# Xjh-UCAS/TAM-TR

Measured on AMD Instinct MI355X. Metric: images/sec fwd+bwd @640x640 bs=16/GPU, higher is better.
Workload: dtype bf16

## Files before the change

### include/tamtr_hip.h

```cpp
#ifndef TAMTR_HIP_H
#define TAMTR_HIP_H

#include <stdint.h>

#ifdef __cplusplus
extern "C" {
#endif

#define TAMTR_F32 0
#define TAMTR_BF16 1

#define TAMTR_OK 0
#define TAMTR_EINVAL (-1)
#define TAMTR_EUNSUP (-2)
#define TAMTR_ELAUNCH (-3)

int tamtr_abi_version(void);

int tamtr_maxsigmoid_gate_fwd(const void* x, const float* gk, const float* bias, const void* v, void* out, float* aw,
                              int32_t* arg, int B, int nh, int hc, int HW, int T, float scale, int dtype, void* stream);

int tamtr_maxsigmoid_gate_bwd(const void* dout, const void* x, const float* gk, const void* v, const float* aw,
                              const int32_t* arg, void* dx, void* dv, float* dlogit, int B, int nh, int hc, int HW, int T,
                              float scale, int dtype, void* stream);
// ... 13 lines not shown
int tamtr_msdeform_attn_fwd(const void* value, const int32_t* shapes_host, const float* loc, const float* aw, void* out,
                            int B, int L, int M, int D, int Q, int nl, int P, int dtype, void* stream);

int tamtr_msdeform_attn_bwd(const void* gout, const void* value, const int32_t* shapes_host, const float* loc,
                            const float* aw, float* gvalue, float* gloc, float* gaw, int B, int L, int M, int D, int Q,
                            int nl, int P, int dtype, void* stream);

int tamtr_msdeform_attn_bwd_sorted(const void* gout, const void* value, const int32_t* shapes_host, const float* loc,
                                   const float* aw, void* gvalue, float* gloc, float* gaw, float* colw, int B, int L, int M,
                                   int D, int Q, int nl, int P, long long ldg, int dtype, void* stream);

int tamtr_contrastive_logits_fwd(const void* x, const float* w, const float* logit_scale, const float* bias, float* logits,
                                 float* xinv, float* winv, int B, int Q, int K, int C, int dtype, void* stream);

int tamtr_contrastive_bwd_slabs(int Q);
int tamtr_contrastive_logits_bwd(const float* g, const void* x, const float* w, const float* logit_scale, const float* xinv,
                                 const float* winv, void* dx, float* dwhat, int B, int Q, int K, int C, int dtype,
                                 void* stream);

int tamtr_linear_bf16(const void* X, const void* W, const float* bias, void* Y, int M, int N, int K, void* stream);

int tamtr_selfattn_fwd(const void* q, const void* k, const void* v, const uint32_t* mask_bits, void* o, float* lse, int B,
                       int Q, int nh, int dh, int ldq, int ldk, int ldv, int dtype, void* stream);
int tamtr_selfattn_bwd(const void* go, const void* q, const void* k, const void* v, const void* o, const float* lse,
                       const uint32_t* mask_bits, void* gq, void* gk, void* gv, float* delta_ws, int B, int Q, int nh, int dh,
                       int ldq, int ldk, int ldv, int dtype, void* stream);

int tamtr_selective_scan_chunk(void);
int tamtr_selective_scan_fwd(const float* u, const float* delta, const float* A, const float* Bm, const float* Cm,
                             const float* D, const float* dbias, float* y, float* hstate, int B, int K, int Dk, int N, int L,
                             int xmode, void* stream);
int tamtr_selective_scan_bwd_slabs(int Dk);
int tamtr_selective_scan_row_sums(void);
int tamtr_selective_scan_bwd(const float* gy, const float* u, const float* delta, const float* A, const float* Bm,
                             const float* Cm, const float* D, const float* dbias, const float* hstate, float* gu,
                             float* gdelta, float* grow, float* gB, float* gC, float* ws, int B, int K, int Dk, int N, int L,
                             int xmode, void* stream);

int tamtr_selective_scan_dtproj_fwd(const void* u, const float* dtr, const float* Wdt, const float* A, const float* Bm,
                                    const float* Cm, const float* D, const float* dbias, void* y, float* hstate, int B, int K,
                                    int Dk, int N, int R, int L, int xmode, int planes_bf16, void* stream);
int tamtr_selective_scan_dtproj_bwd(const void* gy, const void* u, const float* dtr, const float* Wdt, const float* A,
                                    const float* Bm, const float* Cm, const float* D, const float* dbias, const float* hstate,
                                    void* gu, void* gdelta_ws, float* gdtr, float* grow, float* gB, float* gC, float* ws, int B,
                                    int K, int Dk, int N, int R, int L, int xmode, int bf16_flags, void* stream);

int tamtr_lsap_assign(const float* cost, const int32_t* group_sizes_host, int bs, int nq, int G, int64_t* batch_idx,
                      int64_t* query_idx, int64_t* gt_idx, void* stream);

int tamtr_cpam_fwd(const void* x, const void* p, void* out, float* s2, int32_t* arg, int B, int C, int H, int W, int dtype,
                   void* stream);

int tamtr_cpam_bwd(const void* gout, const void* x, const void* p, const float* s2, const int32_t* arg, void* dx_direct,
                   void* du_ws, void* dp, int B, int C, int H, int W, int dtype, void* stream);

int tamtr_cpam_cl_fwd(const void* x, void* p, uint8_t* code, void* out, float* s2, int32_t* arg, int B, int C, int H, int W, int dtype, void* stream);
int tamtr_cpam_cl_bwd(const void* gout, const void* x, const void* p, const uint8_t* code, const float* s2, const int32_t* arg, void* dxd_ws,
                      void* du_ws, void* dp_ws, void* dx, int B, int C, int H, int W, int dtype, void* stream);

int tamtr_dwconv_silu_cross_fwd(const void* x, long long x_pixel_stride, const float* weight, const float* bias, void* u2, int B,
                                int D, int H, int W, int dtype, int plane_dtype, void* stream);
int tamtr_dwconv_tiles(int H, int W);
int tamtr_dwconv_silu_cross_bwd(const void* g2, const void* x, long long x_pixel_stride, const float* weight, const float* bias,
                                void* gx, long long gx_pixel_stride, float* ws, int B, int D, int H, int W, int dtype, int plane_dtype,
                                void* stream);

int tamtr_cross_merge_fwd(const void* y4, float* ymT, int B, int D, int H, int W, int plane_dtype, void* stream);
int tamtr_cross_merge_bwd(const float* gymT, void* g2, int B, int D, int H, int W, int plane_dtype, void* stream);

int tamtr_ln_gate_blocks(long long ntok);
int tamtr_ln_gate_fwd(const float* x, const void* xz, long long xz_token_stride, const float* gamma, const float* beta, void* out,
                      float* stats, long long ntok, int D, float eps, int dtype, void* stream);
int tamtr_ln_gate_bwd(const void* gout, const float* x, const void* xz, long long xz_token_stride, const float* gamma,
                      const float* beta, const float* stats, float* gx, void* gxz, float* partials, long long ntok, int D, int dtype,
                      void* stream);

int tamtr_sum_n(const void* const* src, int n, void* out, long long n_elems, int dtype, void* stream);

int tamtr_colsum_blocks(long long M);
int tamtr_colsum_bf16(const void* X, float* partial, long long M, int N, void* stream);
int tamtr_slab_sum_rows(const void* in, float* out, int R, long long C, int dtype, void* stream);
int tamtr_dw_slices(long long M, int N, int K);
int tamtr_dw_bf16(const void* dY, const void* X, float* part, int with_db, long long M, int N, int K, void* stream);
int tamtr_fold_add(const float* g4, const void* m0, const void* m1, float* out, int B, long long n, int dtype, void* stream);

int tamtr_layernorm_fwd(const void* x, const float* gamma, const float* beta, void* out, float* stats, long long ntok, int D,
                        float eps, int dtype, void* stream);
int tamtr_layernorm_bwd(const void* gout, const void* x, const float* gamma, const float* stats, void* gx, float* partials,
                        long long ntok, int D, int dtype, void* stream);

int tamtr_bn_slices(int B, int HW);
int tamtr_bn_act_fwd(const void* x, const float* gamma, const float* beta, float* running_mean, float* running_var, void* y,
                     float* mean_rstd, float* partials, int B, int C, int HW, float eps, float momentum, int act, int dtype, void* stream);
int tamtr_bn_act_bwd(const void* gy, const void* x, const float* gamma, const float* beta, const float* mean_rstd, void* gx,
                     float* ggamma, float* gbeta, float* partials, int B, int C, int HW, int act, int dtype, void* stream);

int tamtr_bncl_blocks(long long N, int C, int dtype);
int tamtr_bncl_act_fwd(const void* x, const float* gamma, const float* beta, float* running_mean, float* running_var, const void* residual,
                       void* y, float* mean_rstd, float* partials, long long N, int C, float eps, float momentum, int act, int dtype,
                       void* stream);
int tamtr_bncl_stats(const void* x, float* running_mean, float* running_var, float* mean_rstd, float* partials, long long N, int C, float eps,
                     float momentum, int dtype, void* stream);
int tamtr_bncl2_act_fwd(const void* x1, const float* gamma1, const float* beta1, float* running_mean1, float* running_var1, const void* x2,
                        const float* gamma2, const float* beta2, float* running_mean2, float* running_var2, void* y, float* mean_rstd,
                        float* partials, long long N, int C, float eps, float momentum, int act, int dtype, void* stream);
int tamtr_bncl2_act_bwd(const void* gy, long long ldgy, const void* x1, const void* x2, const float* gamma1, const float* beta1,
                        const float* gamma2, const float* beta2, const float* mean_rstd, void* gx1, void* gx2, float* ggamma1, float* gbeta1,
                        float* ggamma2, float* gbeta2, float* partials, long long N, int C, int act, int dtype, void* stream);
int tamtr_bncl_act_bwd(const void* gy, long long ldgy, const void* x, const float* gamma, const float* beta, const float* mean_rstd,
                       void* gx, float* ggamma, float* gbeta, float* partials, long long N, int C, int act, int dtype, void* stream);
int tamtr_bncl_act_down2_fwd(const void* x, const float* gamma, const float* beta, float* running_mean, float* running_var, void* y,
                             float* mean_rstd, float* partials, int B, int H, int W, int C, float eps, float momentum, int act, int dtype,
                             void* stream);
int tamtr_bncl_act_down2_bwd(const void* gy, long long ldgy, const void* x, const float* gamma, const float* beta, const float* mean_rstd,
                             void* gx, float* ggamma, float* gbeta, float* partials, int B, int H, int W, int C, int act, int dtype,
                             void* stream);

int tamtr_relayout(const void* src, void* dst, int B, int C, int HW, int ld, int to_nhwc, int dtype, void* stream);
int tamtr_resample2(const void* src, void* dst, int B, int H, int W, int C, int mode, int dtype, void* stream);
int tamtr_copy_rows(const void* src, long long lds, void* dst, long long ldd, long long N, int C, int dtype, void* stream);
int tamtr_cat_rows(const void* const* src, const long long* lds, const int* C, int n, void* dst, long long ldd, long long N, int dtype,
                   void* stream);

int tamtr_maxpool_out(int n, int k, int s, int p);
int tamtr_maxpool_fwd(const void* x, void* y, uint8_t* code, int B, int C, int H, int W, int k, int s, int p, int nhwc, int dtype,
                      void* stream);
int tamtr_maxpool_bwd(const void* gy, const uint8_t* code, const void* addend, void* gx, int B, int C, int H, int W, int k, int s, int p, int nhwc, int dtype,
                      void* stream);

int tamtr_img_augment_u8(const uint8_t* src, const double* inv_affine, const uint8_t* luts, const int32_t* flags, float* out, int B,
                         int SH, int SW, int H, int W, int border, void* stream);

int tamtr_optim_chunk(void);
int tamtr_optim_step(const void* const* p, const void* const* m, const void* const* v, const void* const* e, const void* const* shadow, float* step,
                     const long long* numel,
                     const unsigned char* group, const int* chunk_tensor, const long long* chunk_off, const void* const* grads, int ntensors,
                     int nchunks, float* partial, float* normcoef, const float* lr, const float* wd, int ngroups, float beta1, float beta2, float eps,
                     float max_norm, float ema_decay, int do_ema, void* stream);

int tamtr_xproj_dw_slices(int L);
int tamtr_xproj_fwd(const void* u2, const void* wcat, float* dtr, float* Bs, float* Cs, int B, int D, int L, int R, int plane_dtype, void* stream);
int tamtr_xproj_bwd_dx(const void* gu, const float* gdtr, const float* gB, const float* gC, const void* wT, void* gu2, int B, int D, int L, int R,
                       int plane_dtype, void* stream);
int tamtr_xproj_bwd_dw(const void* u2, const float* gdtr, const float* gB, const float* gC, float* part, int B, int D, int L, int R, int plane_dtype,
                       void* stream);

int tamtr_detr_blocks(int rows_per_layer);
int tamtr_detr_layers_fwd(const float* pb, const float* ps, const float* gt_bboxes, const long long* gt_cls, const long long* li, const long long* bi,
                          const long long* si, const long long* gi, int Lr, int B, int nq, int nc, int n, long long* tgt, float* score, float* pair_l1,
                          float* pair_riou, float* partial, float g_class, float g_bbox, float g_giou, float* out, void* stream);
int tamtr_detr_layers_bwd(const float* pb, const float* ps, const float* gt_bboxes, const long long* li, const long long* bi, const long long* si,
                          const long long* gi, const long long* tgt, const float* score, const float* up, int Lr, int B, int nq, int nc, int n,
                          float g_class, float g_bbox, float g_giou, float* gpb, float* gps, void* stream);
int tamtr_detr_match_cost(const float* ps, const float* pb, const float* gt_bboxes, const long long* gt_cls, long long rows, int nc, int G, float g_class,
                          float g_bbox, float g_giou, float alpha, float gamma, float* C, void* stream);

int tamtr_bncl_act_seg_fwd(const void* x, const float* gamma, const float* beta, float* running_mean, float* running_var, void* y, long long seg_rows,
                           long long seg_pitch, float* mean_rstd, float* partials, long long N, int C, float eps, float momentum, int act, int dtype,
                           void* stream);
int tamtr_bncl_act_seg_bwd(const void* gy, long long seg_rows, long long seg_pitch, const void* x, const float* gamma, const float* beta,
                           const float* mean_rstd, void* gx, float* ggamma, float* gbeta, float* partials, long long N, int C, int act, int dtype,
                           void* stream);

int tamtr_box_refine_fwd(const float* delta, const float* ref, float* out, long long n, void* stream);
int tamtr_box_refine_bwd(const float* gout, const float* out, const float* ref, float* gdelta, float* gref, long long n, void* stream);

// ... 129 lines not shown
```

### tam-tr_amd/_lib.py

```python
import ctypes
import os
from ctypes import c_float, c_int, c_longlong, c_void_p

_HERE = os.path.dirname(os.path.abspath(__file__))
LIB_PATH = os.environ.get('TAMTR_HIP_LIB') or os.path.join(_HERE, 'csrc', 'libtamtr_hip.so')
ABI_VERSION = 36

F32, BF16 = 0, 1
_ERR = {-1: 'TAMTR_EINVAL (bad argument)', -2: 'TAMTR_EUNSUP (shape/dtype outside what the kernels are built for)',
        -3: 'TAMTR_ELAUNCH (HIP launch error)'}


class TamtrHipError(RuntimeError):
    pass


_P, _I, _F, _LL, _D = c_void_p, c_int, c_float, c_longlong, ctypes.c_double
_SIGS = {
    'tamtr_abi_version': [],
    'tamtr_maxsigmoid_gate_fwd': [_P, _P, _P, _P, _P, _P, _P, _I, _I, _I, _I, _I, _F, _I, _P],
    'tamtr_maxsigmoid_gate_bwd': [_P, _P, _P, _P, _P, _P, _P, _P, _P, _I, _I, _I, _I, _I, _F, _I, _P],
    'tamtr_msdeform_attn_fwd': [_P, _P, _P, _P, _P, _I, _I, _I, _I, _I, _I, _I, _I, _P],
    'tamtr_msdeform_attn_bwd': [_P, _P, _P, _P, _P, _P, _P, _P, _I, _I, _I, _I, _I, _I, _I, _I, _P],
    'tamtr_msdeform_attn_bwd_sorted': [_P, _P, _P, _P, _P, _P, _P, _P, _P, _I, _I, _I, _I, _I, _I, _I, _LL, _I, _P],
    'tamtr_contrastive_logits_fwd': [_P, _P, _P, _P, _P, _P, _P, _I, _I, _I, _I, _I, _P],
    'tamtr_contrastive_logits_bwd': [_P, _P, _P, _P, _P, _P, _P, _P, _I, _I, _I, _I, _I, _P],
    'tamtr_contrastive_bwd_slabs': [_I],
    'tamtr_linear_bf16': [_P, _P, _P, _P, _I, _I, _I, _P],
    'tamtr_selfattn_fwd': [_P, _P, _P, _P, _P, _P, _I, _I, _I, _I, _I, _I, _I, _I, _P],
    'tamtr_selfattn_bwd': [_P] * 11 + [_I, _I, _I, _I, _I, _I, _I, _I, _P],
    'tamtr_selective_scan_chunk': [],
    'tamtr_selective_scan_fwd': [_P, _P, _P, _P, _P, _P, _P, _P, _P, _I, _I, _I, _I, _I, _I, _P],
    'tamtr_selective_scan_bwd_slabs': [_I],
    'tamtr_selective_scan_row_sums': [],
    'tamtr_selective_scan_bwd': [_P] * 15 + [_I, _I, _I, _I, _I, _I, _P],
    'tamtr_selective_scan_dtproj_fwd': [_P] * 10 + [_I] * 8 + [_P],
    'tamtr_selective_scan_dtproj_bwd': [_P] * 17 + [_I] * 8 + [_P],
    'tamtr_lsap_assign': [_P, _P, _I, _I, _I, _P, _P, _P, _P],
    'tamtr_img_augment_u8': [_P, _P, _P, _P, _P, _I, _I, _I, _I, _I, _I, _P],
    'tamtr_cpam_fwd': [_P, _P, _P, _P, _P, _I, _I, _I, _I, _I, _P],
    'tamtr_cpam_cl_fwd': [_P, _P, _P, _P, _P, _P, _I, _I, _I, _I, _I, _P],
    'tamtr_cpam_bwd': [_P] * 8 + [_I, _I, _I, _I, _I, _P],
    'tamtr_cpam_cl_bwd': [_P] * 10 + [_I, _I, _I, _I, _I, _P],
    'tamtr_dwconv_silu_cross_fwd': [_P, _LL, _P, _P, _P, _I, _I, _I, _I, _I, _I, _P],
    'tamtr_dwconv_tiles': [_I, _I],
    'tamtr_cross_merge_fwd': [_P, _P, _I, _I, _I, _I, _I, _P],
    'tamtr_cross_merge_bwd': [_P, _P, _I, _I, _I, _I, _I, _P],
    'tamtr_ln_gate_blocks': [_LL],
    'tamtr_bn_slices': [_I, _I],
    'tamtr_maxpool_out': [_I, _I, _I, _I],
    'tamtr_maxpool_fwd': [_P, _P, _P, _I, _I, _I, _I, _I, _I, _I, _I, _I, _P],
    'tamtr_maxpool_bwd': [_P, _P, _P, _P, _I, _I, _I, _I, _I, _I, _I, _I, _I, _P],
    'tamtr_sum_n': [_P, _I, _P, _LL, _I, _P],
    'tamtr_colsum_blocks': [_LL],
    'tamtr_colsum_bf16': [_P, _P, _LL, _I, _P],
    'tamtr_fold_add': [_P, _P, _P, _P, _I, _LL, _I, _P],
    'tamtr_slab_sum_rows': [_P, _P, _I, _LL, _I, _P],
    'tamtr_dw_slices': [_LL, _I, _I],
    'tamtr_dw_bf16': [_P, _P, _P, _I, _LL, _I, _I, _P],
    'tamtr_graph_capture_census': [_P, _P, _I],
    'tamtr_box_refine_fwd': [_P, _P, _P, _LL, _P],
    'tamtr_box_refine_bwd': [_P, _P, _P, _P, _P, _LL, _P],
    'tamtr_bncl_act_seg_fwd': [_P, _P, _P, _P, _P, _P, _LL, _LL, _P, _P, _LL, _I, _F, _F, _I, _I, _P],
    'tamtr_bncl_act_seg_bwd': [_P, _LL, _LL, _P, _P, _P, _P, _P, _P, _P, _P, _LL, _I, _I, _I, _P],
    'tamtr_detr_blocks': [_I],
    'tamtr_detr_layers_fwd': [_P] * 8 + [_I] * 5 + [_P] * 5 + [_F, _F, _F, _P, _P],
    'tamtr_detr_layers_bwd': [_P] * 10 + [_I] * 5 + [_F, _F, _F, _P, _P, _P],
    'tamtr_detr_match_cost': [_P, _P, _P, _P, _LL, _I, _I, _F, _F, _F, _F, _F, _P, _P],
    'tamtr_xproj_dw_slices': [_I],
    'tamtr_xproj_fwd': [_P, _P, _P, _P, _P, _I, _I, _I, _I, _I, _P],
    'tamtr_xproj_bwd_dx': [_P, _P, _P, _P, _P, _P, _I, _I, _I, _I, _I, _P],
    'tamtr_xproj_bwd_dw': [_P, _P, _P, _P, _P, _I, _I, _I, _I, _I, _P],
    'tamtr_optim_chunk': [],
    'tamtr_optim_step': [_P] * 11 + [_I, _I, _P, _P, _P, _P, _I, _F, _F, _F, _F, _F, _I, _P],
    'tamtr_resample2': [_P, _P, _I, _I, _I, _I, _I, _I, _P],
    'tamtr_cat_rows': [_P, _P, _P, _I, _P, _LL, _LL, _I, _P],
    'tamtr_copy_rows': [_P, _LL, _P, _LL, _LL, _I, _I, _P],
    'tamtr_relayout': [_P, _P, _I, _I, _I, _I, _I, _I, _P],
    'tamtr_bncl_blocks': [_LL, _I, _I],
    'tamtr_bncl_act_fwd': [_P, _P, _P, _P, _P, _P, _P, _P, _P, _LL, _I, _F, _F, _I, _I, _P],
    'tamtr_bncl_stats': [_P, _P, _P, _P, _P, _LL, _I, _F, _F, _I, _P],
    'tamtr_bn_finalize': [_P, _P, _P, _P, _I, _I, _F, _F, _P],
    'tamtr_conv3x3_tiles': [_I, _I, _I],
    'tamtr_conv3x3_pack_weight': [_P, _P, _I, _I, _I, _P],
    'tamtr_conv3x3_cl_stats_fwd': [_P, _LL, _P, _P, _P, _P, _P, _P, _I, _I, _I, _I, _I, _F, _F, _P],
    'tamtr_maxsigmoid_gate_cl_fwd': [_P, _LL, _P, _P, _P, _P, _P, _P, _P, _P, _P, _P, _P, _P, _I, _I, _I, _I, _I, _F, _I, _P],
    'tamtr_bncl2_act_fwd': [_P, _P, _P, _P, _P, _P, _P, _P, _P, _P, _P, _P, _P, _LL, _I, _F, _F, _I, _I, _P],
    'tamtr_bncl2_act_bwd': [_P, _LL, _P, _P, _P, _P, _P, _P, _P, _P, _P, _P, _P, _P, _P, _P, _LL, _I, _I, _I, _P],
    'tamtr_bncl_act_bwd': [_P, _LL, _P, _P, _P, _P, _P, _P, _P, _P, _LL, _I, _I, _I, _P],
    'tamtr_bncl_act_down2_fwd': [_P, _P, _P, _P, _P, _P, _P, _P, _I, _I, _I, _I, _F, _F, _I, _I, _P],
    'tamtr_bncl_act_down2_bwd': [_P, _LL, _P, _P, _P, _P, _P, _P, _P, _P, _I, _I, _I, _I, _I, _I, _P],
    'tamtr_bn_act_fwd': [_P, _P, _P, _P, _P, _P, _P, _P, _I, _I, _I, _F, _F, _I, _I, _P],
    'tamtr_bn_act_bwd': [_P, _P, _P, _P, _P, _P, _P, _P, _P, _I, _I, _I, _I, _I, _P],
    'tamtr_layernorm_fwd': [_P, _P, _P, _P, _P, _LL, _I, _F, _I, _P],
    'tamtr_layernorm_bwd': [_P, _P, _P, _P, _P, _P, _LL, _I, _I, _P],
    'tamtr_ln_gate_fwd': [_P, _P, _LL, _P, _P, _P, _P, _LL, _I, _F, _I, _P],
    'tamtr_ln_gate_bwd': [_P, _P, _P, _LL, _P, _P, _P, _P, _P, _P, _LL, _I, _I, _P],
    'tamtr_dwconv_silu_cross_bwd': [_P, _P, _LL, _P, _P, _P, _LL, _P, _I, _I, _I, _I, _I, _I, _P],
    'tamtr_detect_postprocess': [_P, _I, _I, _I, _I, _P, _F, _F, _I, _F, _P, _I, _P, _P, _P, _P],
    'tamtr_val_postprocess_match': [_P, _I, _I, _I, _I, _F, _F, _F, _I, _F, _P, _P, _P, _I, _P, _P, _P, _P, _P],
    'tamtr_val_confusion': [_P, _P, _I, _I, _I, _P, _P, _P, _I, _P, _F, _F, _P, _P],
    'tamtr_val_ap_tile': [],
    'tamtr_val_ap_curves': [_P, _P, _P, _I, _I, _P, _I] + [_P] * 10 + [_P],
    'tamtr_text_embed': [_P, _P, _P, _P, _LL, _I, _I, _I, _P],
    'tamtr_linear_f32': [_P, _P, _P, _P, _P, _I, _I, _I, _I, _P],
    'tamtr_text_pool_project': [_P, _P, _P, _P, _P, _P, _I, _I, _I, _I, _F, _I, _P],
    'tamtr_bytetrack_update': [_P, _P, _I, _I, _P, _P, _P, _P, _P, _I, _F, _F, _F, _D, _I, _P, _P, _P, _I, _P],
    'tamtr_bytetrack_workspace_bytes': [_I, _I],
    'tamtr_botsort_update': [_P, _P, _P, _I, _I, _P, _P, _P, _P, _P, _I, _F, _F, _F, _D, _I, _P, _P, _P, _I, _P],
    'tamtr_botsort_reid_update': [_P, _P, _P, _P, _I, _I, _P, _P, _P, _P, _P, _P, _I, _I, _F, _F, _F, _D, _I, _F, _D, _P, _P, _P, _I, _P],
    'tamtr_botsort_reid_workspace_bytes': [_I, _I],
    'tamtr_reid_rows': [_P, _I, _P, _P, _I, _I, _I, _I, _P, _P],
    'tamtr_gmc_workspace_bytes': [_I, _I, _I],
    'tamtr_gmc_workspace_offset': [_I, _I, _I, _I],
    'tamtr_gmc_state_bytes': [_I, _I],
    'tamtr_gmc_estimate': [_P, _P, _P, _I, _I, _I, _P, _P, _P, _P, _P, _P, _I, _I, _P],
    'tamtr_bytetrack_update_streams': [_P, _P, _I, _I, _I, _P, _P, _P, _P, _P, _I, _F, _F, _F, _D, _I, _P, _P, _P, _I, _P],
    'tamtr_bytetrack_streams_workspace_bytes': [_I, _I, _I],
    'tamtr_botsort_update_streams': [_P, _P, _P, _I, _I, _I, _P, _P, _P, _P, _P, _I, _F, _F, _F, _D, _I, _P, _P, _P, _I, _P],
    'tamtr_botsort_reid_update_streams': [_P, _P, _P, _P, _I, _I, _I, _P, _P, _P, _P, _P, _P, _I, _I, _F, _F, _F, _D, _I, _F, _D, _P, _P, _P, _I,
                                          _P],
    'tamtr_botsort_reid_streams_workspace_bytes': [_I, _I, _I],
    'tamtr_gmc_estimate_streams': [_P, _P, _P, _I, _I, _I, _I, _P, _P, _P, _P, _P, _P, _I, _I, _P],
    'tamtr_val_coco_match': [_P, _P, _I, _I, _I, _P, _P, _P, _I, _P, _P, _I, _P, _P, _P, _P, _I, _P],
    'tamtr_val_coco_workspace_bytes': [_I, _I, _I],
    'tamtr_val_coco_accumulate': [_P, _P, _P, _I, _I, _P, _P, _I, _P, _P, _P, _P, _P],
    'tamtr_mot_update': [_P, _P, _P, _P, _I, _I, _I, _I, _D, _P, _P, _P, _P, _P, _I, _I, _P, _I, _P],
    'tamtr_mot_end_sequence': [_I, _P, _P, _P, _P, _I, _I, _I, _P, _I, _P],
    'tamtr_mot_workspace_bytes': [_I, _I, _I, _I, _I],
    'tamtr_hota_update': [_P, _P, _P, _P, _I, _I, _I, _I, _D, _D, _P, _P, _P, _I, _P],
    'tamtr_hota_end_sequence': [_P, _D, _I, _I, _I, _I, _P, _P, _P, _I, _P],
    'tamtr_hota_workspace_bytes': [_I, _I, _I],
    'tamtr_mot_update_streams': [_P, _P, _P, _P, _I, _I, _I, _I, _I, _D, _P, _P, _P, _P, _P, _P, _I, _I, _P, _I, _P],
    'tamtr_mot_end_streams': [_I, _I, _P, _P, _P, _P, _P, _P, _I, _I, _P, _I, _P],
    'tamtr_mot_streams_workspace_bytes': [_I, _I, _I, _I, _I, _I],
    'tamtr_hota_update_streams': [_P, _P, _P, _P, _I, _I, _I, _I, _I, _D, _D, _P, _P, _P, _P, _I, _P],
    'tamtr_hota_end_streams': [_P, _D, _I, _I, _P, _I, _I, _I, _P, _P, _P, _I, _P],
    'tamtr_hota_streams_workspace_bytes': [_I, _I, _I, _I],
    'tamtr_trackmap_update': [_P, _P, _P, _P, _I, _I, _I, _I, _D, _P, _P, _P, _I, _P],
    'tamtr_trackmap_end_sequence': [_P, _I, _D, _I, _P, _P, _P, _I, _P],
    'tamtr_trackmap_workspace_bytes': [_I, _I, _I, _I, _I, _I],
    'tamtr_tta_view': [_P, _P, _I, _I, _I, _I, _I, _I, _I, _I, _P],
# ... 78 lines not shown
```

### tam-tr_amd/csrc/dwgrad.hip

```cpp
#include "common.h"

namespace {

constexpr int DW_T = 256;
constexpr int DW_ROWS = 64;
constexpr int DW_RB = 128;
constexpr int DW_SMAX = 64;
constexpr int DW_MIN_ROWS = 256;
constexpr int DW_FILL = 512;

__device__ __forceinline__ uint32_t dswz(int row, int chunk) { return (uint32_t)row * DW_RB + (uint32_t)((chunk ^ ((row ^ (row >> 3)) & 7)) << 4); }

template <int TN, int TK>
__global__ __launch_bounds__(DW_T, 2) void dw_bf16_kernel(const bf16_t* __restrict__ dY, const bf16_t* __restrict__ X, float* __restrict__ part,
                                                           int with_db, long long M, int N, int K, long long rps, int n_tiles, int k_tiles, int S, long long pitch) {
  extern __shared__ __attribute__((aligned(16))) unsigned char smem[];
  constexpr int ST_BYTES = (TN + TK) * DW_RB;
  constexpr int NI = TN / 64, KI = TK / 64;
  const int tid = threadIdx.x, lane = tid & 63, wave = tid >> 6;
  const int wn = wave >> 1, wk = wave & 1;
  const int lr = lane & 31, lh = lane >> 5;
  const int xcd = blockIdx.x & 7, slot = blockIdx.x >> 3;
  int sl, nt, kt;
  if (S >= 8) {
    const int tiles = n_tiles * k_tiles, t = slot % tiles;
    sl = (slot / tiles) * 8 + xcd; nt = t / k_tiles; kt = t % k_tiles;
  } else {
    const int unit = (slot / k_tiles) * 8 + xcd;
    sl = unit / n_tiles; nt = unit % n_tiles; kt = slot % k_tiles;
  }
  if (sl >= S) return;
  const int n0 = nt * TN, k0 = kt * TK;
  const long long m_lo = (long long)sl * rps;
  const long long m_hi = m_lo + rps < M ? m_lo + rps : M;
  const int nst = (int)((m_hi - m_lo + DW_ROWS - 1) / DW_ROWS);

  const bool isY = tid < TN, has_task = tid < TN + TK;
  const int u = isY ? tid : tid - TN;
  const int cpr = (isY ? TN : TK) / 8;
  const int c = u % cpr, rg = u / cpr;
  const int ld = isY ? N : K;
  const int col = (isY ? n0 : k0) + 8 * c;
  const bool col_ok = has_task && col < ld;
  const bf16_t* src = (isY ? dY : X) + (col_ok ? col : 0);
  const long long mrow = m_lo + rg * 8;
  unsigned char* sdst = smem + (isY ? 0 : TN * DW_RB);
  const bool do_db = with_db && kt == 0 && isY;

  uint4 r[8];
  unsigned live = 0;
  float colacc[8];
#pragma unroll
  for (int j = 0; j < 8; ++j) colacc[j] = 0.f;

  auto g_load = [&](int st) {
    const long long m = mrow + (long long)st * DW_ROWS;
    live = 0;
#pragma unroll
    for (int i = 0; i < 8; ++i) {
      const bool in = m + i < m_hi;
      r[i] = *reinterpret_cast<const uint4*>(src + (size_t)(in ? m + i : m_hi - 1) * ld);
      live |= (col_ok && in ? 1u : 0u) << i;
    }
  };
  auto s_store = [&](int stage) {
    if (!has_task) return;
#pragma unroll
    for (int i = 0; i < 8; ++i)
      if (!((live >> i) & 1)) r[i] = make_uint4(0, 0, 0, 0);
    if (do_db) {
#pragma unroll
      for (int i = 0; i < 8; ++i) {
        const uint32_t d[4] = {r[i].x, r[i].y, r[i].z, r[i].w};
#pragma unroll
        for (int q = 0; q < 4; ++q) {
          colacc[2 * q] += __uint_as_float(d[q] << 16);
          colacc[2 * q + 1] += __uint_as_float(d[q] & 0xffff0000u);
        }
      }
    }
    unsigned char* base = sdst + stage * ST_BYTES;
#pragma unroll
    for (int q = 0; q < 4; ++q) {
      uint32_t lo[4], hi[4];
#pragma unroll
      for (int e = 0; e < 4; ++e) {
        const uint32_t a = q == 0 ? r[2 * e].x : q == 1 ? r[2 * e].y : q == 2 ? r[2 * e].z : r[2 * e].w;
        const uint32_t b = q == 0 ? r[2 * e + 1].x : q == 1 ? r[2 * e + 1].y : q == 2 ? r[2 * e + 1].z : r[2 * e + 1].w;
        lo[e] = (a & 0xffffu) | (b << 16);
        hi[e] = (a >> 16) | (b & 0xffff0000u);
      }
      *reinterpret_cast<uint4*>(base + dswz(8 * c + 2 * q, rg)) = make_uint4(lo[0], lo[1], lo[2], lo[3]);
      *reinterpret_cast<uint4*>(base + dswz(8 * c + 2 * q + 1, rg)) = make_uint4(hi[0], hi[1], hi[2], hi[3]);
    }
  };

  f32x16 acc[NI][KI];
#pragma unroll
  for (int a = 0; a < NI; ++a)
#pragma unroll
    for (int b = 0; b < KI; ++b)
#pragma unroll
      for (int q = 0; q < 16; ++q) acc[a][b][q] = 0.f;

  g_load(0);
  s_store(0);
  __syncthreads();
  for (int st = 0; st < nst; ++st) {
    const int cur = st & 1;
    if (st + 1 < nst) g_load(st + 1);
    const unsigned char* sy = smem + cur * ST_BYTES;
    const unsigned char* sx = sy + TN * DW_RB;
#pragma unroll
    for (int ks = 0; ks < DW_ROWS / 16; ++ks) {
      const int ch = ks * 2 + lh;
      s16x8 fy[NI], fx[KI];
#pragma unroll
      for (int i = 0; i < NI; ++i) fy[i] = *reinterpret_cast<const s16x8*>(sy + dswz(wn * (TN / 2) + i * 32 + lr, ch));
#pragma unroll
      for (int j = 0; j < KI; ++j) fx[j] = *reinterpret_cast<const s16x8*>(sx + dswz(wk * (TK / 2) + j * 32 + lr, ch));
#pragma unroll
      for (int i = 0; i < NI; ++i)
#pragma unroll
        for (int j = 0; j < KI; ++j) acc[i][j] = __builtin_amdgcn_mfma_f32_32x32x16_bf16(fy[i], fx[j], acc[i][j], 0, 0, 0);
    }
    if (st + 1 < nst) {
      s_store(cur ^ 1);
      __syncthreads();
    }
  }

  float* out = part + (size_t)sl * pitch;
#pragma unroll
  for (int i = 0; i < NI; ++i)
#pragma unroll
    for (int j = 0; j < KI; ++j) {
      const int k = k0 + wk * (TK / 2) + j * 32 + lr;
#pragma unroll
      for (int q = 0; q < 16; ++q) {
        const int n = n0 + wn * (TN / 2) + i * 32 + (q & 3) + 8 * (q >> 2) + 4 * lh;
        if (n < N && k < K) out[(size_t)n * K + k] = acc[i][j][q];
      }
    }

  if (kt == 0) {
    float* red = reinterpret_cast<float*>(smem);
    __syncthreads();
    if (do_db) {
#pragma unroll
      for (int j = 0; j < 8; ++j) red[rg * TN + 8 * c + j] = colacc[j];
    }
    __syncthreads();
    if (tid < TN && n0 + tid < N) {
      float s = 0.f;
      if (with_db) {
#pragma unroll
        for (int g = 0; g < 8; ++g) s += red[g * TN + tid];
      }
      out[(size_t)N * K + n0 + tid] = s;
    }
  }
}

struct DwPlan {
  int tn, tk, n_tiles, k_tiles, S;
  long long rps;
};

long long dw_rows_per_slice(long long M, int S) { return ((M + S - 1) / S + DW_ROWS - 1) / DW_ROWS * DW_ROWS; }

bool dw_plan(long long M, int N, int K, DwPlan* p) {
  if (M <= 0 || N <= 0 || K <= 0 || N % 16 || K % 16 || N > 16384 || K > 16384 || M > (1LL << 40)) return false;
  long long smax = M / DW_MIN_ROWS;
  smax = smax < 1 ? 1 : smax > DW_SMAX ? DW_SMAX : smax;
  int tn = N >= 128 ? 128 : 64, tk = K >= 128 ? 128 : 64;
  auto tiles = [&]() { return (long long)((N + tn - 1) / tn) * ((K + tk - 1) / tk); };
  if (tiles() * smax < DW_FILL / 2) tn = tk = 64;
  const long long t = tiles();
  long long S = (DW_FILL + t - 1) / t;
  S = S < 1 ? 1 : S > smax ? smax : S;
  for (;;) {
    const long long rows = dw_rows_per_slice(M, (int)S), s2 = (M + rows - 1) / rows;
    if (s2 == S) break;
    S = s2;
  }
  p->tn = tn; p->tk = tk;
  p->n_tiles = (N + tn - 1) / tn; p->k_tiles = (K + tk - 1) / tk;
  p->S = (int)S;
  p->rps = dw_rows_per_slice(M, (int)S);
  return true;
}

}

extern "C" int tamtr_dw_slices(long long M, int N, int K) {
  DwPlan p;
  return dw_plan(M, N, K, &p) ? p.S : 0;
}

extern "C" int tamtr_dw_bf16(const void* dY, const void* X, float* part, int with_db, long long M, int N, int K, void* stream) {
  if (!dY || !X || !part || M <= 0 || N <= 0 || K <= 0) return TAMTR_EINVAL;
  DwPlan p;
  if (!dw_plan(M, N, K, &p)) return TAMTR_EUNSUP;
  if (((uintptr_t)dY | (uintptr_t)X | (uintptr_t)part) % 16) return TAMTR_EUNSUP;
  const long long pitch = (long long)N * K + (N + 3) / 4 * 4;
  const int groups = p.S >= 8 ? (p.S + 7) / 8 * p.n_tiles * p.k_tiles : (p.S * p.n_tiles + 7) / 8 * p.k_tiles;
  const dim3 grid((unsigned)groups * 8);
  const size_t lds = (size_t)2 * (p.tn + p.tk) * DW_RB;
#define LAUNCH_DW(TN_, TK_)                                                                                                       \
  hipLaunchKernelGGL((dw_bf16_kernel<TN_, TK_>), grid, dim3(DW_T), lds, (hipStream_t)stream, (const bf16_t*)dY, (const bf16_t*)X, \
                     part, with_db, M, N, K, p.rps, p.n_tiles, p.k_tiles, p.S, pitch)
  if (p.tn == 128 && p.tk == 128) LAUNCH_DW(128, 128);
  else if (p.tn == 128) LAUNCH_DW(128, 64);
  else if (p.tk == 128) LAUNCH_DW(64, 128);
  else LAUNCH_DW(64, 64);
#undef LAUNCH_DW
  return tamtr_launch_status();
}
```

### tam-tr_amd/ops.py

```python
import ctypes
import math

import torch

from . import _lib
from ._lib import call, dtype_code, ptr, require_gpu, stream_ptr
import os as _os

_PROJ_CONV_LIB = _os.environ.get('TAMTR_PROJ_CONV') == 'miopen'

_I, _F = ctypes.c_int, ctypes.c_float


def _c(t):
    return t if t.is_contiguous() else t.contiguous()


def _is_cl(t):
    return t.dim() == 4 and not t.is_contiguous() and t.is_contiguous(memory_format=torch.channels_last)


def is_cl(t):
    return _is_cl(t)

# ... 373 lines not shown
        D = N // M
        Q = loc32.shape[1]
        gout = _c(gout.to(torch.bfloat16))
        gloc, gaw = torch.empty_like(loc32), torch.empty_like(aw32)
        colw = torch.empty(B, Q, M, device=gout.device, dtype=torch.float32)
        gvalue = torch.empty(B * L, N, device=gout.device, dtype=torch.bfloat16)
        call('tamtr_msdeform_attn_bwd_sorted', ptr(gout), ptr(value), ctypes.cast(sh, ctypes.c_void_p), ptr(loc32), ptr(aw32),
             ptr(gvalue), ptr(gloc), ptr(gaw), ptr(colw), B, L, M, D, Q, nl, P, N, dtype_code(value), stream_ptr())
        gx = _linear_bf16_dx(gvalue, w16).view(B, L, K) if ctx.needs_input_grad[0] else None
        gw = dw_splitk(gvalue, x2).to(w_dt) if ctx.needs_input_grad[1] else None
        gb = (gout.view(B * Q, M, D).float() * colw.view(B * Q, M, 1)).sum(0).view(N).to(b_dt) if ctx.needs_input_grad[2] else None
        return gx, gw, gb, None, gloc.to(loc_dt), gaw.to(aw_dt), None


def value_proj_msda_ok(x, lin, n_heads, Q, P):
    K, N = lin.in_features, lin.out_features
    return (x.is_cuda and x.dtype == torch.bfloat16 and x.dim() == 3 and lin.bias is not None and N % n_heads == 0 and K % 128 == 0 and N % 128 == 0
            and msda_sorted_ok(Q, P, N // n_heads) and not _MSDA_ATOMICS and _os.environ.get('TAMTR_VALUE_BIAS') != 'colsum')


def value_proj_msda(x, lin, n_heads, shapes, loc, aw):
    return _ValueProjMSDA.apply(x, lin.weight, lin.bias, [tuple(int(v) for v in s) for s in shapes], loc, aw, int(n_heads))


class _ContrastiveLogits(torch.autograd.Function):
    @staticmethod
    def forward(ctx, x, w, logit_scale, bias):
        require_gpu(x, w, logit_scale, bias)
        B, Q, C = x.shape
        K = w.shape[1]
        x = _c(x)
        w32 = _c(w.float())
        ls, bi = _c(logit_scale.float().reshape(1)), _c(bias.float().reshape(1))
        logits = torch.empty(B, Q, K, device=x.device, dtype=torch.float32)
        xinv = torch.empty(B, Q, device=x.device, dtype=torch.float32)
        winv = torch.empty(B, K, device=x.device, dtype=torch.float32)
        call('tamtr_contrastive_logits_fwd', ptr(x), ptr(w32), ptr(ls), ptr(bi), ptr(logits), ptr(xinv), ptr(winv), B, Q, K, C,
             dtype_code(x), stream_ptr())
        ctx.save_for_backward(x, w32, ls, bi, logits, xinv, winv)
        ctx.cfg = (w.dtype, logit_scale.dtype, logit_scale.shape, bias.dtype, bias.shape)
        return logits

    @staticmethod
    def backward(ctx, g):
        x, w32, ls, bi, logits, xinv, winv = ctx.saved_tensors
        w_dt, ls_dt, ls_shape, b_dt, b_shape = ctx.cfg
        B, Q, C = x.shape
        K = w32.shape[1]
        g = _c(g.float())
        dx = torch.empty_like(x)
        if K > 16:
            _atomic_fallback(f'the contrastive head backward sums d(what) with LDS atomics for K = {K} > 16 prompts (csrc/contrastive.hip)')
        slabs = _lib.lib().tamtr_contrastive_bwd_slabs(Q)
        dwhat = torch.empty(B, slabs, K, C, device=x.device, dtype=torch.float32)
        call('tamtr_contrastive_logits_bwd', ptr(g), ptr(x), ptr(w32), ptr(ls), ptr(xinv), ptr(winv), ptr(dx), ptr(dwhat), B, Q, K,
             C, dtype_code(x), stream_ptr())
        dwhat = dwhat.sum(1) if slabs > 1 else dwhat[:, 0]
        what = w32 * winv.unsqueeze(-1)
        dw = winv.unsqueeze(-1) * (dwhat - (dwhat * what).sum(-1, keepdim=True) * what)
        dls = (g * (logits - bi)).sum().reshape(ls_shape).to(ls_dt)
        dbias = g.sum().reshape(b_shape).to(b_dt)
        return dx, dw.to(w_dt), dls, dbias


def contrastive_logits(x, w, logit_scale, bias):
    return _ContrastiveLogits.apply(x, w, logit_scale, bias)


_SPLIT_MAX = int(_os.environ.get('TAMTR_SPLITK_MAX', '64'))


def _split_count(M, min_rows=2048, max_split=None):
    max_split = _SPLIT_MAX if max_split is None else max_split
    S = 1
    while S < max_split and M % (2 * S) == 0 and M // (2 * S) >= min_rows:
        S *= 2
    return S


_BMM_F32_OUT = None

_DW_OWN = _os.environ.get('TAMTR_DW_OWN') != '0'
_DW_OWN_MAX_ROWS = 8192


def _dw_own_slices(g2, x2):
    if not (_DW_OWN and g2.is_cuda and x2.is_cuda and g2.dtype == torch.bfloat16 and x2.dtype == torch.bfloat16 and g2.dim() == 2 and x2.dim() == 2
            and g2.shape[0] == x2.shape[0] and 0 < g2.shape[0] < _DW_OWN_MAX_ROWS and g2.is_contiguous() and x2.is_contiguous()
            and g2.data_ptr() % 16 == 0 and x2.data_ptr() % 16 == 0):
        return 0
    return _lib.lib().tamtr_dw_slices(g2.shape[0], g2.shape[1], x2.shape[1])


def _dw_own(g2, x2, S, with_db):
    M, N = g2.shape
    K = x2.shape[1]
    part = torch.empty(S, N * K + N, device=g2.device, dtype=torch.float32)
    call('tamtr_dw_bf16', ptr(g2), ptr(x2), ptr(part), int(with_db), M, N, K, stream_ptr())
    tot = slab_sum(part)
    return tot[:N * K].view(N, K), tot[N * K:]


def dw_splitk(g2, x2, min_rows=2048):
    M, N = g2.shape
    K = x2.shape[1]
    S = _dw_own_slices(g2, x2)
    if S:
        return _dw_own(g2, x2, S, False)[0]
    S = _split_count(M, min_rows)
    if S == 1:
        return (g2.t() @ x2).float()
    a, b = g2.view(S, M // S, N).transpose(1, 2), x2.view(S, M // S, K)
    global _BMM_F32_OUT
    if _BMM_F32_OUT is not False and N % 8 == 0 and K % 8 == 0:
        try:
            out = torch.bmm(a, b, out_dtype=torch.float32)
            _BMM_F32_OUT = True
            return slab_sum(out)
        except (NotImplementedError, RuntimeError, TypeError):
            if _BMM_F32_OUT:
                raise
            _BMM_F32_OUT = False
    return slab_sum(torch.bmm(a, b))


def slab_sum(t):
    R = t.shape[0]
    C = t.numel() // max(R, 1)
    if not (t.is_cuda and t.dtype in (torch.float32, torch.bfloat16) and t.is_contiguous() and R > 0 and C % 4 == 0 and t.data_ptr() % 16 == 0):
        return t.float().sum(0)
    if R == 1:
        return t[0].float()
    out = torch.empty(t.shape[1:], device=t.device, dtype=torch.float32)
    call('tamtr_slab_sum_rows', ptr(t), ptr(out), R, C, dtype_code(t), stream_ptr())
    return out


def colsum(g2):
    M, N = g2.shape
    if g2.is_cuda and g2.dtype == torch.bfloat16 and M >= 4096 and N % 8 == 0 and N <= 2048 and 256 % (N // 8) == 0 and g2.is_contiguous():
        nblk = _lib.lib().tamtr_colsum_blocks(M)
        part = torch.empty(nblk, N, device=g2.device, dtype=torch.float32)
        call('tamtr_colsum_bf16', ptr(g2), ptr(part), M, N, stream_ptr())
        return slab_sum(part)
    if g2.is_cuda and g2.dtype in (torch.float32, torch.bfloat16) and N % 4 == 0:
        return slab_sum(_c(g2))
    return g2.sum(0, dtype=torch.float32)


def bf16_shadow(p):
    s = getattr(p, '_tamtr_bf16', None)
    if s is not None:
        base = getattr(p, '_tamtr_alias_of', p)
        if s._tamtr_version == base._version and s.device == p.device and s.shape == p.shape:
            return s
    return None


def bf16_of(p):
    if p.dtype == torch.bfloat16:
        return p
    s = bf16_shadow(p)
    return s if s is not None else p.to(torch.bfloat16)


KERNEL_EVENTS = {}


def _a16(t):
    return t if t is None or t.data_ptr() % 16 == 0 else t.clone()


def _linear_bf16_fwd(x2, w16, b32):
    M, K = x2.shape
    N = w16.shape[0]
    y = torch.empty(M, N, device=x2.device, dtype=torch.bfloat16)
    x2, w16, b32 = _a16(x2), _a16(w16), _a16(b32)
    rec = KERNEL_EVENTS.get('tamtr_linear_bf16')
    if rec is not None:
        e0, e1 = torch.cuda.Event(enable_timing=True), torch.cuda.Event(enable_timing=True)
        e0.record()
# ... 2293 lines not shown
```

Baseline: 219.2.

## Route tall weight-gradient GEMMs to own split-K kernel with transposed LDS reads

```diff
diff --git a/include/tamtr_hip.h b/include/tamtr_hip.h
--- a/include/tamtr_hip.h
+++ b/include/tamtr_hip.h
@@ -119,6 +119,11 @@
 int tamtr_slab_sum_rows(const void* in, float* out, int R, long long C, int dtype, void* stream);
 int tamtr_dw_slices(long long M, int N, int K);
 int tamtr_dw_bf16(const void* dY, const void* X, float* part, int with_db, long long M, int N, int K, void* stream);
+int tamtr_dw_tall_plan(long long M, int N, int K);
+int tamtr_dw_tall_routed(long long M, int N, int K);
+int tamtr_dw_tall_bf16(const void* dY, const void* X, float* part, int with_db, long long M, int N, int K, void* stream);
+int tamtr_dw_tall_try_bf16(const void* dY, const void* X, float* part, int with_db, long long M, int N, int K, int S, int tn, int tk,
+                           int tr, void* stream);
 int tamtr_fold_add(const float* g4, const void* m0, const void* m1, float* out, int B, long long n, int dtype, void* stream);
 
 int tamtr_layernorm_fwd(const void* x, const float* gamma, const float* beta, void* out, float* stats, long long ntok, int D,
diff --git a/tam-tr_amd/_lib.py b/tam-tr_amd/_lib.py
--- a/tam-tr_amd/_lib.py
+++ b/tam-tr_amd/_lib.py
@@ -58,6 +58,10 @@
     'tamtr_slab_sum_rows': [_P, _P, _I, _LL, _I, _P],
     'tamtr_dw_slices': [_LL, _I, _I],
     'tamtr_dw_bf16': [_P, _P, _P, _I, _LL, _I, _I, _P],
+    'tamtr_dw_tall_plan': [_LL, _I, _I],
+    'tamtr_dw_tall_routed': [_LL, _I, _I],
+    'tamtr_dw_tall_bf16': [_P, _P, _P, _I, _LL, _I, _I, _P],
+    'tamtr_dw_tall_try_bf16': [_P, _P, _P, _I, _LL, _I, _I, _I, _I, _I, _I, _P],
     'tamtr_graph_capture_census': [_P, _P, _I],
     'tamtr_box_refine_fwd': [_P, _P, _P, _LL, _P],
     'tamtr_box_refine_bwd': [_P, _P, _P, _P, _P, _LL, _P],
diff --git a/tam-tr_amd/csrc/dwgrad.hip b/tam-tr_amd/csrc/dwgrad.hip
--- a/tam-tr_amd/csrc/dwgrad.hip
+++ b/tam-tr_amd/csrc/dwgrad.hip
@@ -11,12 +11,25 @@
 
 __device__ __forceinline__ uint32_t dswz(int row, int chunk) { return (uint32_t)row * DW_RB + (uint32_t)((chunk ^ ((row ^ (row >> 3)) & 7)) << 4); }
 
-template <int TN, int TK>
+__device__ __forceinline__ uint32_t tswz(int row, int chunk) { return (uint32_t)row * 256 + (uint32_t)((chunk ^ (((row & 3) << 2) | ((row >> 2) & 3))) << 4); }
+
+typedef __attribute__((address_space(3))) s16x4 lds_s16x4;
+
+__device__ __forceinline__ s16x8 tr_frag(const unsigned char* rows, int c0, int lane) {
+  const int g = lane >> 4, q = (lane >> 2) & 3, p = lane & 3;
+  const int row = 8 * (g >> 1) + q, chunk = (c0 >> 3) + 2 * (g & 1) + (p >> 1);
+  const s16x4 lo = __builtin_amdgcn_ds_read_tr16_b64_v4i16((lds_s16x4*)(rows + tswz(row, chunk) + 8 * (p & 1)));
+  const s16x4 hi = __builtin_amdgcn_ds_read_tr16_b64_v4i16((lds_s16x4*)(rows + tswz(row + 4, chunk) + 8 * (p & 1)));
+  return __builtin_shufflevector(lo, hi, 0, 1, 2, 3, 4, 5, 6, 7);
+}
+
+template <int TN, int TK, bool TR>
 __global__ __launch_bounds__(DW_T, 2) void dw_bf16_kernel(const bf16_t* __restrict__ dY, const bf16_t* __restrict__ X, float* __restrict__ part,
                                                            int with_db, long long M, int N, int K, long long rps, int n_tiles, int k_tiles, int S, long long pitch) {
   extern __shared__ __attribute__((aligned(16))) unsigned char smem[];
   constexpr int ST_BYTES = (TN + TK) * DW_RB;
   constexpr int NI = TN / 64, KI = TK / 64;
+  static_assert(!TR || (TN == 128 && TK == 128), "the row image has 256-byte rows");
   const int tid = threadIdx.x, lane = tid & 63, wave = tid >> 6;
   const int wn = wave >> 1, wk = wave & 1;
   const int lr = lane & 31, lh = lane >> 5;
@@ -65,9 +78,11 @@
   };
   auto s_store = [&](int stage) {
     if (!has_task) return;
-#pragma unroll
-    for (int i = 0; i < 8; ++i)
-      if (!((live >> i) & 1)) r[i] = make_uint4(0, 0, 0, 0);
+    if (!TR || live != 0xffu) {
+#pragma unroll
+      for (int i = 0; i < 8; ++i)
+        if (!((live >> i) & 1)) r[i] = make_uint4(0, 0, 0, 0);
+    }
     if (do_db) {
 #pragma unroll
       for (int i = 0; i < 8; ++i) {
@@ -80,6 +95,11 @@
       }
     }
     unsigned char* base = sdst + stage * ST_BYTES;
+    if constexpr (TR) {
+#pragma unroll
+      for (int i = 0; i < 8; ++i) *reinterpret_cast<uint4*>(base + tswz(8 * rg + i, c)) = r[i];
+      return;
+    }
 #pragma unroll
     for (int q = 0; q < 4; ++q) {
       uint32_t lo[4], hi[4];
@@ -115,10 +135,17 @@
     for (int ks = 0; ks < DW_ROWS / 16; ++ks) {
       const int ch = ks * 2 + lh;
       s16x8 fy[NI], fx[KI];
-#pragma unroll
-      for (int i = 0; i < NI; ++i) fy[i] = *reinterpret_cast<const s16x8*>(sy + dswz(wn * (TN / 2) + i * 32 + lr, ch));
-#pragma unroll
-      for (int j = 0; j < KI; ++j) fx[j] = *reinterpret_cast<const s16x8*>(sx + dswz(wk * (TK / 2) + j * 32 + lr, ch));
+      if constexpr (TR) {
+#pragma unroll
+        for (int i = 0; i < NI; ++i) fy[i] = tr_frag(sy + ks * 16 * 256, wn * (TN / 2) + i * 32, lane);
+#pragma unroll
+        for (int j = 0; j < KI; ++j) fx[j] = tr_frag(sx + ks * 16 * 256, wk * (TK / 2) + j * 32, lane);
+      } else {
+#pragma unroll
+        for (int i = 0; i < NI; ++i) fy[i] = *reinterpret_cast<const s16x8*>(sy + dswz(wn * (TN / 2) + i * 32 + lr, ch));
+#pragma unroll
+        for (int j = 0; j < KI; ++j) fx[j] = *reinterpret_cast<const s16x8*>(sx + dswz(wk * (TK / 2) + j * 32 + lr, ch));
+      }
 #pragma unroll
       for (int i = 0; i < NI; ++i)
 #pragma unroll
@@ -165,20 +192,16 @@
 struct DwPlan {
   int tn, tk, n_tiles, k_tiles, S;
   long long rps;
+  bool tr = false;
 };
 
 long long dw_rows_per_slice(long long M, int S) { return ((M + S - 1) / S + DW_ROWS - 1) / DW_ROWS * DW_ROWS; }
 
-bool dw_plan(long long M, int N, int K, DwPlan* p) {
-  if (M <= 0 || N <= 0 || K <= 0 || N % 16 || K % 16 || N > 16384 || K > 16384 || M > (1LL << 40)) return false;
-  long long smax = M / DW_MIN_ROWS;
-  smax = smax < 1 ? 1 : smax > DW_SMAX ? DW_SMAX : smax;
-  int tn = N >= 128 ? 128 : 64, tk = K >= 128 ? 128 : 64;
-  auto tiles = [&]() { return (long long)((N + tn - 1) / tn) * ((K + tk - 1) / tk); };
-  if (tiles() * smax < DW_FILL / 2) tn = tk = 64;
-  const long long t = tiles();
-  long long S = (DW_FILL + t - 1) / t;
-  S = S < 1 ? 1 : S > smax ? smax : S;
+bool dw_shape_ok(long long M, int N, int K) { return !(M <= 0 || N <= 0 || K <= 0 || N % 16 || K % 16 || N > 16384 || K > 16384 || M > (1LL << 40)); }
+
+long long dw_pitch(int N, int K) { return (long long)N * K + (N + 3) / 4 * 4; }
+
+void dw_settle(long long M, int tn, int tk, int N, int K, long long S, DwPlan* p) {
   for (;;) {
     const long long rows = dw_rows_per_slice(M, (int)S), s2 = (M + rows - 1) / rows;
     if (s2 == S) break;
@@ -188,7 +211,77 @@
   p->n_tiles = (N + tn - 1) / tn; p->k_tiles = (K + tk - 1) / tk;
   p->S = (int)S;
   p->rps = dw_rows_per_slice(M, (int)S);
+}
+
+bool dw_plan(long long M, int N, int K, DwPlan* p) {
+  if (!dw_shape_ok(M, N, K)) return false;
+  long long smax = M / DW_MIN_ROWS;
+  smax = smax < 1 ? 1 : smax > DW_SMAX ? DW_SMAX : smax;
+  int tn = N >= 128 ? 128 : 64, tk = K >= 128 ? 128 : 64;
+  auto tiles = [&]() { return (long long)((N + tn - 1) / tn) * ((K + tk - 1) / tk); };
+  if (tiles() * smax < DW_FILL / 2) tn = tk = 64;
+  const long long t = tiles();
+  long long S = (DW_FILL + t - 1) / t;
+  S = S < 1 ? 1 : S > smax ? smax : S;
+  dw_settle(M, tn, tk, N, K, S, p);
   return true;
+}
+
+constexpr long long DW_TALL_PART_MAX = 64LL << 20;
+constexpr int DW_TALL_PART_DIV = 3;
+constexpr int DW_TALL_FILL = 512;
+
+bool dw_tall_plan(long long M, int N, int K, DwPlan* p) {
+  if (!dw_shape_ok(M, N, K)) return false;
+  long long cap = M * (long long)(N + K) * 2 / DW_TALL_PART_DIV;
+  cap = cap > DW_TALL_PART_MAX ? DW_TALL_PART_MAX : cap;
+  long long smax = (M + DW_MIN_ROWS - 1) / DW_MIN_ROWS;
+  if (dw_rows_per_slice(M, (int)smax) < DW_MIN_ROWS) smax = M / DW_MIN_ROWS;
+  const long long sbytes = cap / (dw_pitch(N, K) * 4);
+  smax = smax > sbytes ? sbytes : smax;
+  smax = smax < 1 ? 1 : smax;
+  int tn = N >= 128 ? 128 : 64, tk = K >= 128 ? 128 : 64;
+  auto tiles = [&]() { return (long long)((N + tn - 1) / tn) * ((K + tk - 1) / tk); };
+  if (tiles() == 1 && smax < DW_TALL_FILL / 2) tn = tk = 64;
+  const long long t = tiles();
+  long long S = (DW_TALL_FILL + t - 1) / t;
+  S = S < 1 ? 1 : S > smax ? smax : S;
+  dw_settle(M, tn, tk, N, K, S, p);
+  p->tr = tn == 128 && tk == 128;
+  return true;
+}
+
+struct DwRoute {
+  long long M;
+  int N, K;
+};
+constexpr DwRoute DW_TALL_ROUTES[] = {
+    {25600, 128, 128},
+    {102400, 64, 64},  {102400, 64, 128}, {102400, 128, 128},
+    {102400, 128, 256}, {102400, 256, 256},
+    {409600, 128, 128}, {409600, 128, 256}, {409600, 128, 384}, {409600, 128, 512},
+    {409600, 512, 128},
+    {1638400, 128, 64},
+};
+
+int dw_launch(const DwPlan& p, const void* dY, const void* X, float* part, int with_db, long long M, int N, int K, void* stream) {
+  if (((uintptr_t)dY | (uintptr_t)X | (uintptr_t)part) % 16) return TAMTR_EUNSUP;
+  const long long pitch = dw_pitch(N, K);
+  const long long groups = p.S >= 8 ? (long long)(p.S + 7) / 8 * p.n_tiles * p.k_tiles : ((long long)p.S * p.n_tiles + 7) / 8 * p.k_tiles;
+  if (groups * 8 > 0x7fffffffLL) return TAMTR_EUNSUP;
+  const dim3 grid((unsigned)groups * 8);
+  const size_t lds = (size_t)2 * (p.tn + p.tk) * DW_RB;
+#define LAUNCH_DW(TN_, TK_, TR_)                                                                                                            \
+  hipLaunchKernelGGL((dw_bf16_kernel<TN_, TK_, TR_>), grid, dim3(DW_T), lds, (hipStream_t)stream, (const bf16_t*)dY, (const bf16_t*)X, part, \
+                     with_db, M, N, K, p.rps, p.n_tiles, p.k_tiles, p.S, pitch)
+  if (p.tn == 128 && p.tk == 128 && p.tr) LAUNCH_DW(128, 128, true);
+  else if (p.tn == 128 && p.tk == 128) LAUNCH_DW(128, 128, false);
+  else if (p.tn == 128 && p.tk == 64) LAUNCH_DW(128, 64, false);
+  else if (p.tn == 64 && p.tk == 128) LAUNCH_DW(64, 128, false);
+  else if (p.tn == 64 && p.tk == 64) LAUNCH_DW(64, 64, false);
+  else return TAMTR_EUNSUP;
+#undef LAUNCH_DW
+  return tamtr_launch_status();
 }
 
 }
@@ -202,18 +295,35 @@
   if (!dY || !X || !part || M <= 0 || N <= 0 || K <= 0) return TAMTR_EINVAL;
   DwPlan p;
   if (!dw_plan(M, N, K, &p)) return TAMTR_EUNSUP;
-  if (((uintptr_t)dY | (uintptr_t)X | (uintptr_t)part) % 16) return TAMTR_EUNSUP;
-  const long long pitch = (long long)N * K + (N + 3) / 4 * 4;
-  const int groups = p.S >= 8 ? (p.S + 7) / 8 * p.n_tiles * p.k_tiles : (p.S * p.n_tiles + 7) / 8 * p.k_tiles;
-  const dim3 grid((unsigned)groups * 8);
-  const size_t lds = (size_t)2 * (p.tn + p.tk) * DW_RB;
-#define LAUNCH_DW(TN_, TK_)                                                                                                       \
-  hipLaunchKernelGGL((dw_bf16_kernel<TN_, TK_>), grid, dim3(DW_T), lds, (hipStream_t)stream, (const bf16_t*)dY, (const bf16_t*)X, \
-                     part, with_db, M, N, K, p.rps, p.n_tiles, p.k_tiles, p.S, pitch)
-  if (p.tn == 128 && p.tk == 128) LAUNCH_DW(128, 128);
-  else if (p.tn == 128) LAUNCH_DW(128, 64);
-  else if (p.tk == 128) LAUNCH_DW(64, 128);
-  else LAUNCH_DW(64, 64);
-#undef LAUNCH_DW
-  return tamtr_launch_status();
-}
+  return dw_launch(p, dY, X, part, with_db, M, N, K, stream);
+}
+
+extern "C" int tamtr_dw_tall_plan(long long M, int N, int K) {
+  DwPlan p;
+  return dw_tall_plan(M, N, K, &p) ? p.S : 0;
+}
+
+extern "C" int tamtr_dw_tall_routed(long long M, int N, int K) {
+  if (M < 8192) return 0;
+  for (const DwRoute& r : DW_TALL_ROUTES)
+    if (r.M == M && r.N == N && r.K == K) return 1;
+  return 0;
+}
+
+extern "C" int tamtr_dw_tall_bf16(const void* dY, const void* X, float* part, int with_db, long long M, int N, int K, void* stream) {
+  if (!dY || !X || !part || M <= 0 || N <= 0 || K <= 0) return TAMTR_EINVAL;
+  DwPlan p;
+  if (!dw_tall_plan(M, N, K, &p)) return TAMTR_EUNSUP;
+  return dw_launch(p, dY, X, part, with_db, M, N, K, stream);
+}
+
+extern "C" int tamtr_dw_tall_try_bf16(const void* dY, const void* X, float* part, int with_db, long long M, int N, int K, int S, int tn, int tk,
+                                      int tr, void* stream) {
+  if (!dY || !X || !part || M <= 0 || N <= 0 || K <= 0 || S <= 0) return TAMTR_EINVAL;
+  if (!dw_shape_ok(M, N, K) || (tn != 64 && tn != 128) || (tk != 64 && tk != 128) || (tr && (tn != 128 || tk != 128))) return TAMTR_EUNSUP;
+  DwPlan p;
+  dw_settle(M, tn, tk, N, K, S, &p);
+  if (p.S != S) return TAMTR_EUNSUP;
+  p.tr = tr != 0;
+  return dw_launch(p, dY, X, part, with_db, M, N, K, stream);
+}
diff --git a/tam-tr_amd/ops.py b/tam-tr_amd/ops.py
--- a/tam-tr_amd/ops.py
+++ b/tam-tr_amd/ops.py
@@ -479,21 +479,29 @@
 
 _DW_OWN = _os.environ.get('TAMTR_DW_OWN') != '0'
 _DW_OWN_MAX_ROWS = 8192
+_DW_TALL = _os.environ.get('TAMTR_DW_TALL') != '0'
 
 
 def _dw_own_slices(g2, x2):
     if not (_DW_OWN and g2.is_cuda and x2.is_cuda and g2.dtype == torch.bfloat16 and x2.dtype == torch.bfloat16 and g2.dim() == 2 and x2.dim() == 2
-            and g2.shape[0] == x2.shape[0] and 0 < g2.shape[0] < _DW_OWN_MAX_ROWS and g2.is_contiguous() and x2.is_contiguous()
+            and g2.shape[0] == x2.shape[0] and 0 < g2.shape[0] and g2.is_contiguous() and x2.is_contiguous()
             and g2.data_ptr() % 16 == 0 and x2.data_ptr() % 16 == 0):
         return 0
-    return _lib.lib().tamtr_dw_slices(g2.shape[0], g2.shape[1], x2.shape[1])
+    M, N, K = g2.shape[0], g2.shape[1], x2.shape[1]
+    if M < _DW_OWN_MAX_ROWS:
+        return _lib.lib().tamtr_dw_slices(M, N, K)
+    return _lib.lib().tamtr_dw_tall_plan(M, N, K) if _DW_TALL and _dw_tall_routed(M, N, K) else 0
+
+
+def _dw_tall_routed(M, N, K):
+    return bool(_lib.lib().tamtr_dw_tall_routed(M, N, K))
 
 
 def _dw_own(g2, x2, S, with_db):
     M, N = g2.shape
     K = x2.shape[1]
     part = torch.empty(S, N * K + N, device=g2.device, dtype=torch.float32)
-    call('tamtr_dw_bf16', ptr(g2), ptr(x2), ptr(part), int(with_db), M, N, K, stream_ptr())
+    call('tamtr_dw_bf16' if M < _DW_OWN_MAX_ROWS else 'tamtr_dw_tall_bf16', ptr(g2), ptr(x2), ptr(part), int(with_db), M, N, K, stream_ptr())
     tot = slab_sum(part)
     return tot[:N * K].view(N, K), tot[N * K:]
 
```

Result: no change. 220.2, median of 6 (+0.5%).
